# srisarya/nanopore-barcoding-ORC

Measured on AMD Instinct MI355X. Metric: Mreads/s two-round SP5×SP27 demux; % HBM roofline; 1/2/4/8 GPU, higher is better.
Workload: dtype u64

## Files before the change

nanopore-barcoding-orc_amd/csrc/dmx_kernels.hip:

```cpp
#include <algorithm>
#include <cstring>
#include <memory>
#include <type_traits>
#include <utility>
#include <vector>

#include "dmx_device.h"
#include "dmx_internal.h"

namespace dmx {

struct RoundArgs {
    Packed pk;
    const uint64_t* offs;
    const uint32_t* lens;
    const DevPanel* panel;
    const ItemView* items;
    const uint32_t* n_items_dev;
    uint32_t n_items;
    int32_t T;
    int32_t per_task_slot;
    int32_t slot_div;
    Cluster* cl;
    Outcome* outc;
    uint32_t* cl_count;
    uint32_t cl_cap;
    uint32_t* flags;
    unsigned long long* winner;
    int32_t* origin;
    int32_t* lb;
    Window* win;
    uint32_t* win_count;
    uint32_t win_cap;
    uint32_t win_scap;
    Window* win2;
    uint32_t* win2_count;
    uint32_t* diag;
    int32_t band;
    Cand* cand[2];
    uint32_t* cand_count;
    uint32_t cand_cap;
    uint32_t cand_scap;
    int32_t screen;
    Window* tasks;
    uint32_t* task_count;
    uint32_t task_cap;
    uint32_t task_scap;
    const DevPieces* pieces;
    FTask* ftask;
    uint32_t* ftask_count;
    uint32_t ftask_scap;
    uint32_t n_words;
    uint32_t nsb;
    int32_t round;
    uint32_t* cells[4];
};


struct TaskView {
    uint32_t read, n, strand, start, len;
    uint64_t off;
    int o, a;
    bool clean = false;
    uint32_t tag = 0;
    uint32_t sbl = 0;
};

template <class T>
__device__ __forceinline__ __attribute__((address_space(1))) T* sgpr_ptr(T* p) {
    const uint64_t v = reinterpret_cast<uint64_t>(p);
    const uint64_t lo = (uint32_t)__builtin_amdgcn_readfirstlane((uint32_t)v);
    const uint64_t hi = (uint32_t)__builtin_amdgcn_readfirstlane((uint32_t)(v >> 32));
    return reinterpret_cast<__attribute__((address_space(1))) T*>(lo | (hi << 32));
}

typedef unsigned int u32x4_t __attribute__((ext_vector_type(4)));
typedef unsigned int u32x2_t __attribute__((ext_vector_type(2)));
__device__ __forceinline__ void store_cand(__attribute__((address_space(1))) Cand* p, uint32_t i,
                                           const Cand& cd) {
    static_assert(sizeof(Cand) == 40, "Cand layout");
    u32x4_t a, b;
    u32x2_t c;
    __builtin_memcpy(&a, reinterpret_cast<const char*>(&cd), 16);
    __builtin_memcpy(&b, reinterpret_cast<const char*>(&cd) + 16, 16);
    __builtin_memcpy(&c, reinterpret_cast<const char*>(&cd) + 32, 8);
    auto* d = reinterpret_cast<__attribute__((address_space(1))) char*>(p + i);
    *reinterpret_cast<__attribute__((address_space(1))) u32x4_t*>(d) = a;
    *reinterpret_cast<__attribute__((address_space(1))) u32x4_t*>(d + 16) = b;
    *reinterpret_cast<__attribute__((address_space(1))) u32x2_t*>(d + 32) = c;
}

__device__ __forceinline__ void view_off(uint64_t off, TaskView& tv) {
    tv.off = off & kOffMask;
    tv.tag = 0;
    tv.sbl = 0;
}

__device__ __forceinline__ void fetch16t(const Packed& pk, const TaskView& tv, uint32_t p,
                                         uint32_t& codes, uint32_t& nbits, bool load_mask = true) {
    fetch16(pk, tv.off, tv.n, tv.strand, tv.start, p, codes, nbits, load_mask);
}

__device__ __forceinline__ bool empty_view(TaskView& tv) {
    tv.read = 0;
    tv.n = tv.start = tv.len = tv.strand = 0;
    tv.off = kMinOffset;
    tv.o = tv.a = 0;
    return false;
}

__device__ __forceinline__ bool task_view(const RoundArgs& R, uint32_t item, int sub, int A,
                                          TaskView& tv) {
    if (R.items) {
        if (!DMX_BOUND(R.pk.bd, items, item, kBufItem)) return empty_view(tv);
        const ItemView v = R.items[item];
        tv.read = v.read;
        tv.start = v.start;
        tv.len = v.len;
        tv.strand = v.strand;
        if (v.only_adapter >= 0) {
            tv.o = 0;
            tv.a = v.only_adapter;
        } else {
            tv.o = sub / A;
            tv.a = sub % A;
        }
    } else {
        tv.read = item;
        tv.start = 0;
        tv.strand = 0;
        tv.len = R.lens[item];
        tv.o = sub / A;
        tv.a = sub % A;
        if (R.per_task_slot) {
            tv.o = 0;
            tv.a = sub;
        }
    }
    if (!DMX_BOUND(R.pk.bd, reads, tv.read, kBufRead)) return empty_view(tv);
    tv.n = R.lens[tv.read];
    tv.off = R.offs[tv.read];
    if (tv.o) {
        tv.start = tv.n - tv.start - tv.len;
        tv.strand ^= 1u;
    }
    return true;
}

__device__ __forceinline__ uint32_t slot_of(const RoundArgs& R, uint32_t item, int sub) {
    if (R.per_task_slot) return item * (uint32_t)R.T + (uint32_t)sub;
    return R.slot_div ? 2u * item + (uint32_t)(sub >= R.slot_div) : item;
}

constexpr int kPeqStride = kMaxAdapters + 24;
constexpr int kIpeqStride = 9;

struct AdLite {
    int m, k, kk;
    bool front;
// ... 178 lines not shown
        __builtin_amdgcn_wave_barrier();
        if (lane == 0) *cnt = 0;
        __builtin_amdgcn_wave_barrier();
    }
};

__device__ __forceinline__ uint32_t wave_shard() {
    return (blockIdx.x * (kScanBlock / 64) + (threadIdx.x >> 6)) & (uint32_t)(kShards - 1);
}

struct ShardMap {
    uint32_t* pre;
    uint32_t scap;
    __device__ __forceinline__ void load(const uint32_t* counts, uint32_t shard_cap) {
        scap = shard_cap;
        if (threadIdx.x == 0) {
            uint32_t t = 0;
            for (int k = 0; k < kShards; ++k) {
                pre[k] = t;
                t += min(counts[k * kShardStride], shard_cap);
            }
            pre[kShards] = t;
        }
        __syncthreads();
    }
    __device__ __forceinline__ uint32_t total() const { return pre[kShards]; }
    __device__ __forceinline__ uint32_t phys(uint32_t t) const {
        uint32_t s = 0;
#pragma unroll
        for (uint32_t h = kShards / 2; h > 0; h >>= 1)
            if (t >= pre[s + h]) s += h;
        return s * scap + (t - pre[s]);
    }
};

#ifndef DMX_WAVE_CAND_CAP
#define DMX_WAVE_CAND_CAP 32
#endif
#ifndef DMX_WAVE_CAND_FLUSH
#define DMX_WAVE_CAND_FLUSH (DMX_WAVE_CAND_CAP / 2)
#endif
constexpr int kWaveCandCap = DMX_WAVE_CAND_CAP;
constexpr int kWaveWinCap = 64;

struct WaveCandSink {
    WaveStage<Cand, kWaveCandCap> st[2];
};

__device__ __forceinline__ Cand make_cand(const TaskView& tv, uint32_t item, int sub, int iend,
                                          int cost, uint32_t j) {
    Cand c;
    c.item = item;
    c.sub = (uint16_t)sub;
    c.iend = (uint8_t)iend;
    c.cost = (uint8_t)cost;
    c.j = j;
    c.n = tv.n;
    c.start = tv.start;
    c.len = tv.len;
    c.strand = (uint8_t)tv.strand;
    c.o = (uint8_t)tv.o;
    c.a = (uint8_t)tv.a;
    c.clean = tv.clean ? 1 : 0;
    c.off = tv.off | ((uint64_t)tv.tag << kOffBits);
    return c;
}

__device__ __forceinline__ bool viable_lb(int lbk, int lr, int o, int cost) {
    return beats_lb(lbk, lr - 2 * cost, o, cost);
}

template <bool MASK = true>
__device__ __forceinline__ void fetch16s(const Packed& pk, const TaskView& tv, int p,
                                         uint32_t& codes, uint32_t& nbits) {
    p = max(p, -kViewReachPre);
    if (tv.strand == 0) {
        const int64_t g = (int64_t)tv.off + (int64_t)tv.start + p;
        codes = code32(pk, g);
        nbits = (MASK && !tv.clean) ? mask32(pk, g) & 0xFFFFu : 0u;
    } else {
        const int64_t b = (int64_t)tv.off + (int64_t)tv.n - 1 - (int64_t)tv.start - p - 15;
        codes = ~rev_pairs(code32(pk, b));
        nbits = (MASK && !tv.clean) ? __brev(mask32(pk, b)) >> 16 : 0u;
    }
}

struct Chunk16 {
    uint64_t c = 0, m = 0;
};
__device__ __forceinline__ int64_t chunk16_pos(const TaskView& tv, int p) {
    p = max(p, -kViewReachPre);
    const int64_t f = (int64_t)tv.off + (int64_t)tv.start + p;
    const int64_t b = (int64_t)tv.off + (int64_t)tv.n - 1 - (int64_t)tv.start - p - 15;
    return tv.strand ? b : f;
}
__device__ __forceinline__ uint64_t load8(const uint32_t* __restrict__ w, int64_t q,
                                          const Bounds& bd, uint32_t buf) {
#ifdef DMX_DEBUG_BOUNDS
    if (!bchk(bd, q, bd.lo, bd.hi - 1, buf)) return 0ull;
#else
    (void)bd, (void)buf;
#endif
    uint64_t v;
    __builtin_memcpy(&v, w + q, 8);
    return v;
}
template <bool MASK = true>
__device__ __forceinline__ Chunk16 chunk16_load(const Packed& pk, const TaskView& tv, int p) {
    const int64_t g = chunk16_pos(tv, p);
    Chunk16 r;
    r.c = load8(pk.seq, (2 * g) >> 5, pk.bd, kBufSeq);
    if (MASK && !tv.clean) r.m = load8(pk.nmask, g >> 5, pk.bd, kBufMask);
    return r;
}
template <bool MASK = true>
__device__ __forceinline__ void chunk16_codes(const TaskView& tv, int p, const Chunk16& r,
                                              uint32_t& codes, uint32_t& nbits) {
    const int pc = max(p, -kViewReachPre);
    const uint32_t f = (uint32_t)tv.off + tv.start + (uint32_t)pc;
    const uint32_t b = (uint32_t)tv.off + tv.n - 1u - tv.start - (uint32_t)pc - 15u;
    const uint32_t g = tv.strand ? b : f;
    const uint32_t c = (uint32_t)(r.c >> ((2u * g) & 31u));
    codes = tv.strand ? ~rev_pairs(c) : c;
    if (MASK) {
        const uint32_t m = (uint32_t)(r.m >> (g & 31u));
        nbits = tv.strand ? __brev(m) >> 16 : m & 0xFFFFu;
    } else {
        nbits = 0u;
    }
}

__device__ __forceinline__ uint32_t mask32s(const Packed& pk, const TaskView& tv, int p) {
    if (tv.strand == 0) return mask32(pk, (int64_t)tv.off + (int64_t)tv.start + p);
    return __brev(mask32(pk, (int64_t)tv.off + (int64_t)tv.n - 1 - (int64_t)tv.start - p - 31));
}

template <class Sink>
__device__ __forceinline__ void flush_cands(const Sink& sink, const TaskView& tv, uint32_t item,
                                         int sub, int m, int lbk, uint32_t seg, uint64_t cm,
                                         uint64_t c0, uint64_t c1, uint64_t c2) {
    while (cm) {
        const int bit = __ffsll((unsigned long long)cm) - 1;
        cm &= cm - 1;
        const int cost = (int)((c0 >> bit) & 1ull) | ((int)((c1 >> bit) & 1ull) << 1) |
                         ((int)((c2 >> bit) & 1ull) << 2);
        const uint32_t j = seg + (uint32_t)bit;
        if (!viable_lb(lbk, min(m, (int)j + cost), tv.o, cost)) continue;
        const Cand cd = make_cand(tv, item, sub, m, cost, j);
        if (cost <= 3) sink.st[0].push(cd);
        else sink.st[1].push(cd);
    }
}

struct Bytes16 {
    uint32_t w0 = 0, w1 = 0, w2 = 0, w3 = 0;
    __device__ __forceinline__ void put(int q, uint32_t v) {
        const uint32_t sel = (0x03020100u & ~(0xFFu << (8 * (q & 3)))) | (4u << (8 * (q & 3)));
        if (q < 4) w0 = __builtin_amdgcn_perm(v, w0, sel);
        else if (q < 8) w1 = __builtin_amdgcn_perm(v, w1, sel);
        else if (q < 12) w2 = __builtin_amdgcn_perm(v, w2, sel);
        else w3 = __builtin_amdgcn_perm(v, w3, sel);
    }
    __device__ __forceinline__ int get(int q) const {
        const uint32_t x = q < 8 ? (q < 4 ? w0 : w1) : (q < 12 ? w2 : w3);
        return (int)(int8_t)(uint8_t)(x >> (8 * (q & 3)));
    }
};

struct CandOut {
    uint64_t cells = 0, c0 = 0, c1 = 0, c2 = 0;
    uint64_t rows0 = 0, rows1 = 0;
    uint64_t pv = 0, mv = 0;
    uint32_t seg = 0;
    int mlist = -1;
};

__device__ __forceinline__ uint32_t wave_sum(uint32_t v) {
#pragma unroll
    for (int d = 32; d >= 1; d >>= 1) v += __shfl_xor(v, d, 64);
    return v;
}

__device__ __forceinline__ uint32_t wave_excl_scan(uint32_t v, uint32_t& total) {
    const uint32_t lane = threadIdx.x & 63u;
    uint32_t x = v;
#pragma unroll
    for (int d = 1; d < 64; d <<= 1) {
        const uint32_t y = __shfl_up(x, d, 64);
        if (lane >= (uint32_t)d) x += y;
    }
    total = __shfl(x, 63, 64);
    return x - v;
}

__device__ __forceinline__ void emit_cands(const RoundArgs& R, const CandOut& co,
                                           const TaskView& tv, uint32_t item, int sub, int m) {
    const uint32_t n1 = (uint32_t)(__popcll(co.cells & co.c2) + __popcll(co.rows1) +
                                   (co.mlist == 1 ? 1 : 0));
    const uint32_t n0 = (uint32_t)(__popcll(co.cells & ~co.c2) + __popcll(co.rows0) +
                                   (co.mlist == 0 ? 1 : 0));
    uint32_t tot;
    const uint32_t pre = wave_excl_scan(n0 | (n1 << 16), tot);
    if (tot == 0) return;
    const uint32_t sh = wave_shard();
    uint32_t b0 = 0, b1 = 0;
    if ((threadIdx.x & 63u) == 0) {
        if (tot & 0xFFFFu) b0 = atomicAdd(R.cand_count + sh * kShardStride, tot & 0xFFFFu);
        if (tot >> 16) b1 = atomicAdd(R.cand_count + (kShards + sh) * kShardStride, tot >> 16);
    }
    b0 = __builtin_amdgcn_readfirstlane(b0) + (pre & 0xFFFFu);
    b1 = __builtin_amdgcn_readfirstlane(b1) + (pre >> 16);
    __attribute__((address_space(1))) Cand* const cl0 = sgpr_ptr(R.cand[0] + sh * R.cand_scap);
    __attribute__((address_space(1))) Cand* const cl1 = sgpr_ptr(R.cand[1] + sh * R.cand_scap);
    const auto put = [&](int l, const Cand& cd) __attribute__((always_inline)) {
        const uint32_t i = l ? b1++ : b0++;
        if (i < R.cand_scap) store_cand(l ? cl1 : cl0, i, cd);
        else atomicOr(R.flags, 8u);
    };
    uint64_t x = co.cells;
    while (x) {
        const int bit = __ffsll((unsigned long long)x) - 1;
        x &= x - 1;
        const int cost = (int)((co.c0 >> bit) & 1ull) | ((int)((co.c1 >> bit) & 1ull) << 1) |
                         ((int)((co.c2 >> bit) & 1ull) << 2);
        put(cost > 3, make_cand(tv, item, sub, m, cost, co.seg + (uint32_t)bit));
    }
    x = co.rows0 | co.rows1;
    while (x) {
        const int i = __ffsll((unsigned long long)x) - 1;
        x &= x - 1;
        const int cost = col_cost(co.pv, co.mv, i);
        put(cost > 3, make_cand(tv, item, sub, i, cost, tv.len));
    }
    if (co.mlist >= 0)
        put(co.mlist, make_cand(tv, item, sub, m, col_cost(co.pv, co.mv, m), tv.len));
}

template <int HB, class Sink>
__device__ __forceinline__ int scan_task_cand_hb(const RoundArgs& R, const Sink& sink,
                                                 const TaskView& tv, uint32_t item, int sub,
                                                 const uint64_t* peq, int A, AdLite ad,
                                                 const int8_t* acc, const int8_t* pacc,
                                                 uint32_t js, bool real, uint32_t jlo,
                                                 uint32_t jhi, bool lastcol,
                                                 CandOut* out = nullptr) {
    const int m = ad.m;
    const int kk = ad.kk;
    const bool front = ad.front;
    const uint32_t hbit = (uint32_t)(m - 1);

    uint64_t pv = (front && real) ? 0ull : ~0ull, mv = 0ull;
    int d = (front && real) ? 0 : m;
    int lbk = 0;
    bool segset = false;
    uint32_t seg = 0;
    uint64_t cm = 0, c0 = 0, c1 = 0, c2 = 0;

    auto hit = [&](uint32_t j, int dv) __attribute__((always_inline)) {
        bool ok = j >= jlo;
        int L0 = m;
        if (ok && (int)j < m + kk) {
            ok = dv <= (int)pacc[min(m, (int)j + dv)];
            L0 = min(m, (int)j - dv);
            if (ok && !(L0 >= 0 && dv <= (int)acc[L0])) L0 = -1;
        }
        if (ok) {
            if (L0 >= 0) lbk = max(lbk, lb_key(L0 - 3 * dv, tv.o, dv));
            if (!segset) {
                segset = true;
                seg = j;
            }
            const uint64_t bm = 1ull << (j - seg);
            cm |= bm;
            if (dv & 1) c0 |= bm;
            if (dv & 2) c1 |= bm;
            if (dv & 4) c2 |= bm;
        }
    };
    const int e0 = kk + 1;
    int e = d - e0;
#define DMX_CAND_REC(q)                                                                   \
    {                                                                                     \
        myers_step<HB>(eqv(q), pv, mv, e, hbit);                                          \
        hits = __builtin_amdgcn_alignbit(hits, (uint32_t)e, 31);                          \
        dq.put((q), (uint32_t)e);                                                         \
    }
#define DMX_CAND_VISIT(NQ)                                                                \
    while (hits) {                                                                        \
        const int q = (int)__clz(hits) - (32 - (NQ));                                     \
        hits &= ~(0x80000000u >> __clz(hits));                                            \
        hit(p0 + (uint32_t)q + 1u, dq.get(q) + e0);                                    \
    }
#define DMX_CAND_EQ                                                                       \
    const auto eqv = [&](int q) __attribute__((always_inline)) {                          \
        const uint32_t cq = (codes >> (2 * q)) & 3u, nq = (nb >> q) & 1u;                 \
        return peq[(cq | (nq << 2)) * kPeqStride];                                        \
    };

    uint32_t p0 = js;
    Chunk16 nx = chunk16_load(R.pk, tv, (int)p0);
    for (; p0 + 16 <= jhi; p0 += 16) {
        uint32_t codes, nb;
        chunk16_codes(tv, (int)p0, nx, codes, nb);
        if (p0 + 16 < jhi) nx = chunk16_load(R.pk, tv, (int)p0 + 16);
        if (segset && p0 + 16 >= seg + 64) {
            flush_cands(sink, tv, item, sub, m, lbk, seg, cm, c0, c1, c2);
            segset = false;
            cm = c0 = c1 = c2 = 0;
        }
        DMX_CAND_EQ
        uint32_t hits = 0;
        Bytes16 dq;
#pragma unroll
        for (int q = 0; q < 16; ++q) DMX_CAND_REC(q)
        DMX_CAND_VISIT(16)
    }
    if (p0 < jhi) {
        uint32_t codes, nb;
        chunk16_codes(tv, (int)p0, nx, codes, nb);
        if (segset && p0 + 16 >= seg + 64) {
            flush_cands(sink, tv, item, sub, m, lbk, seg, cm, c0, c1, c2);
            segset = false;
            cm = c0 = c1 = c2 = 0;
        }
        DMX_CAND_EQ
        const int cnt = (int)(jhi - p0);
        uint32_t hits = 0;
        Bytes16 dq;
#pragma unroll
        for (int q = 0; q < 16; ++q)
            if (q < cnt) DMX_CAND_REC(q)
        while (hits) {
            const int q = (int)__clz(hits) - (32 - cnt);
            hits &= ~(0x80000000u >> __clz(hits));
            hit(p0 + (uint32_t)q + 1u, dq.get(q) + e0);
        }
    }
    d = e + e0;
#undef DMX_CAND_REC
#undef DMX_CAND_VISIT
#undef DMX_CAND_EQ
    uint64_t rows = 0;
    bool mrow = false;
    const uint32_t len = tv.len;
    if (lastcol && !front) {
        int dd = 0;
        const int ilast = len == 0 ? m : m - 1;
        for (int i = 1; i <= ilast; ++i) {
            dd += (int)((pv >> (i - 1)) & 1ull) - (int)((mv >> (i - 1)) & 1ull);
            if (dd <= (int)acc[i]) {
                if (i < m) rows |= 1ull << i;
                else mrow = true;
                lbk = max(lbk, lb_key(i - 3 * dd, tv.o, dd));
            }
        }
    }
    if (out) {
        uint64_t keep = 0, x = cm;
        while (x) {
            const int bit = __ffsll((unsigned long long)x) - 1;
            x &= x - 1;
            const int cost = (int)((c0 >> bit) & 1ull) | ((int)((c1 >> bit) & 1ull) << 1) |
                             ((int)((c2 >> bit) & 1ull) << 2);
            if (viable_lb(lbk, min(m, (int)(seg + (uint32_t)bit) + cost), tv.o, cost))
                keep |= 1ull << bit;
        }
        out->cells = keep;
        out->c0 = c0;
        out->c1 = c1;
        out->c2 = c2;
        out->seg = seg;
        out->pv = pv;
        out->mv = mv;
        out->rows0 = out->rows1 = 0;
        while (rows) {
            const int i = __ffsll((unsigned long long)rows) - 1;
            rows &= rows - 1;
            const int cost = col_cost(pv, mv, i);
            if (!viable_lb(lbk, i, tv.o, cost)) continue;
            if (cost <= 3) out->rows0 |= 1ull << i;
            else out->rows1 |= 1ull << i;
        }
        out->mlist = -1;
        if (mrow) {
            const int cost = col_cost(pv, mv, m);
            if (viable_lb(lbk, m, tv.o, cost)) out->mlist = cost <= 3 ? 0 : 1;
        }
        return lbk;
    }
    if (cm) flush_cands(sink, tv, item, sub, m, lbk, seg, cm, c0, c1, c2);
    while (rows) {
        const int i = __ffsll((unsigned long long)rows) - 1;
        rows &= rows - 1;
        const int cost = col_cost(pv, mv, i);
        if (!viable_lb(lbk, i, tv.o, cost)) continue;
        const Cand cd = make_cand(tv, item, sub, i, cost, len);
        if (cost <= 3) sink.st[0].push(cd);
        else sink.st[1].push(cd);
    }
    if (mrow) {
        const int cost = col_cost(pv, mv, m);
        if (viable_lb(lbk, m, tv.o, cost)) {
            const Cand cd = make_cand(tv, item, sub, m, cost, len);
            if (cost <= 3) sink.st[0].push(cd);
            else sink.st[1].push(cd);
        }
    }
    return lbk;
}

template <class Sink>
__device__ __forceinline__ int scan_task_cand(const RoundArgs& R, const Sink& sink,
                                              const TaskView& tv, uint32_t item, int sub,
                                              const uint64_t* peq, int A, AdLite ad,
                                              const int8_t* acc, const int8_t* pacc,
                                              uint32_t js, bool real, uint32_t jlo,
                                              uint32_t jhi, bool lastcol,
                                              CandOut* out = nullptr) {
    if (ad.m > 32)
        return scan_task_cand_hb<1, Sink>(R, sink, tv, item, sub, peq, A, ad, acc, pacc, js, real,
                                          jlo, jhi, lastcol, out);
    return scan_task_cand_hb<0, Sink>(R, sink, tv, item, sub, peq, A, ad, acc, pacc, js, real, jlo,
                                      jhi, lastcol, out);
}

#define DMX_CAND_STAGE                                                                    \
    __shared__ Cand s_cand[2][kCandStageCap];                                             \
    __shared__ uint32_t s_ccnt[2], s_cbase[2];                                            \
    if (threadIdx.x < 2) s_ccnt[threadIdx.x] = 0;                                         \
    const uint32_t bsh = blockIdx.x & (uint32_t)(kShards - 1);                           \
    const CandSink sink{{Stage<Cand, kCandStageCap>{s_cand[0], &s_ccnt[0], &s_cbase[0],    \
                                                    R.cand[0] + bsh * R.cand_scap,         \
                                                    R.cand_count + bsh * kShardStride,     \
                                                    R.cand_scap,                           \
                                                    R.flags, 8u},                          \
                         Stage<Cand, kCandStageCap>{s_cand[1], &s_ccnt[1], &s_cbase[1],    \
                                                    R.cand[1] + bsh * R.cand_scap,         \
                                                    R.cand_count +                         \
                                                        (kShards + bsh) * kShardStride,    \
                                                    R.cand_scap, R.flags, 8u}}};

#define DMX_STAGES                                                                        \
    __shared__ Cluster s_cl[BAND ? 1 : kStageCap];                                        \
    __shared__ uint32_t s_clcnt, s_clbase;                                                \
    if (threadIdx.x == 0) s_clcnt = 0;                                                    \
    const Stage<Cluster> st{s_cl, &s_clcnt, &s_clbase, R.cl, R.cl_count, R.cl_cap,        \
                            R.flags, 1u};                                                 \
    __shared__ Cand s_cand[2][BAND ? kCandStageCap : 1];                                  \
    __shared__ uint32_t s_ccnt[2], s_cbase[2];                                            \
    if (threadIdx.x < 2) s_ccnt[threadIdx.x] = 0;                                         \
    const uint32_t bsh = blockIdx.x & (uint32_t)(kShards - 1);                           \
    const CandSink sink{{Stage<Cand, kCandStageCap>{s_cand[0], &s_ccnt[0], &s_cbase[0],    \
                                                    R.cand[0] + bsh * R.cand_scap,         \
                                                    R.cand_count + bsh * kShardStride,     \
                                                    R.cand_scap,                           \
                                                    R.flags, 8u},                          \
                         Stage<Cand, kCandStageCap>{s_cand[1], &s_ccnt[1], &s_cbase[1],    \
                                                    R.cand[1] + bsh * R.cand_scap,         \
                                                    R.cand_count +                         \
                                                        (kShards + bsh) * kShardStride,    \
                                                    R.cand_scap, R.flags, 8u}}};

#define DMX_CLUSTER_STAGE                                                                 \
    __shared__ Cluster s_cl[kStageCap];                                                   \
    __shared__ uint32_t s_clcnt, s_clbase;                                                \
    if (threadIdx.x == 0) s_clcnt = 0;                                                    \
    const Stage<Cluster> st{s_cl, &s_clcnt, &s_clbase, R.cl, R.cl_count, R.cl_cap,        \
                            R.flags, 1u};

template <bool BAND>
__global__ __launch_bounds__(kScanBlock) void scan_kernel(RoundArgs R) {
    __shared__ uint64_t s_peq[8 * kPeqStride];
    __shared__ int8_t s_acc[72 * kMaxAdapters];
    __shared__ int8_t s_pacc[72 * kMaxAdapters];
    __shared__ uint32_t s_amk[kMaxAdapters];
    DMX_STAGES
    load_panel_lds(R.panel, s_peq, s_acc, s_pacc, s_amk);
    __syncthreads();

    const int A = R.panel->n_adapters;
    const int T = R.T;
    const int rpb = kScanBlock / T;
    const int tid = threadIdx.x;
    const uint32_t item = blockIdx.x * (uint32_t)rpb + (uint32_t)(tid / T);
    const int sub = tid % T;
    const uint32_t n_items = R.items ? *R.n_items_dev : R.n_items;
    if (tid < rpb * T && item < n_items) {
        TaskView tv;
// ... 1897 lines not shown
                        hi |= spread_bits_nib(nb >> 8);
                    }
                    uint32_t cm0 = 0xFFFFFFFFu, cm1 = 0xFFFFFFFFu;
                    u16x2 m0 = as_pk(cm0), m1 = as_pk(cm1);
#if DMX_SCREEN_BARE
                    {
                        ScreenState ss{pv0, mv0, pv1, mv1, d0, d1, m0, m1};
                        screen_chunk<DMX_SCREEN_BARE>(qb, lo, hi, q8, qlo, ss, stale);
                        pv0 = ss.pv0, mv0 = ss.mv0, pv1 = ss.pv1, mv1 = ss.mv1;
                        d0 = ss.d0, d1 = ss.d1, m0 = ss.m0, m1 = ss.m1;
                    }
#else
                    if (__builtin_amdgcn_ballot_w64(qlo > 0) == 0) {
#pragma unroll
                        for (int c = 0; c < 16; ++c) {
                            const uint64_t e = *reinterpret_cast<const uint64_t*>(
                                qb + lds_off32(__builtin_amdgcn_ubfe(c < 8 ? lo : hi,
                                                                     4 * (c & 7), 4), q8));
                            myers_step_pk((uint32_t)e, pv0, mv0, d0);
                            myers_step_pk((uint32_t)(e >> 32), pv1, mv1, d1);
                            m0 = __builtin_elementwise_min(m0, d0);
                            m1 = __builtin_elementwise_min(m1, d1);
                        }
                    } else {
#pragma unroll
                        for (int c = 0; c < 16; ++c) {
                            const uint64_t e = *reinterpret_cast<const uint64_t*>(
                                qb + lds_off32(__builtin_amdgcn_ubfe(c < 8 ? lo : hi,
                                                                     4 * (c & 7), 4), q8));
                            myers_step_pk((uint32_t)e, pv0, mv0, d0);
                            myers_step_pk((uint32_t)(e >> 32), pv1, mv1, d1);
                            if (c >= qlo) {
                                m0 = __builtin_elementwise_min(m0, d0);
                                m1 = __builtin_elementwise_min(m1, d1);
                            }
                        }
                    }
#endif
                    cm0 = as_u32(m0);
                    cm1 = as_u32(m1);
#pragma unroll
                    for (int k = 0; k < 4; ++k) {
                        const uint32_t cmk = ((k < 2 ? cm0 : cm1) >> (16 * (k & 1))) & 0xFFFFu;
                        const int tk = max(inR ? thr[k] : -1, inE ? thre[k] : -1);
                        if (((need >> k) & 1u) && !((pass_m >> k) & 1u) && (int)cmk <= tk) {
                            pass_m |= 1u << k;
                            if (inR) end_m &= ~(1u << k);
                        }
                    }
                }
                if (lastc) {
#pragma unroll
                    for (int k = 0; k < 4; ++k) {
                        if (!((need >> k) & 1u) || ((pass_m >> k) & 1u)) continue;
                        const int a = 4 * q + k;
                        if (dPn > (int)s_pimax[a]) continue;
                        const uint32_t par = s_par[a];
                        const int l = (int)(par & 255u), lc = (int)(par >> 24);
                        const uint32_t pvh = ((k < 2 ? pv0 : pv1) >> (16 * (k & 1))) & 0xFFFFu;
                        const uint32_t mvh = ((k < 2 ? mv0 : mv1) >> (16 * (k & 1))) & 0xFFFFu;
                        bool ok = false;
                        int dd = 0;
                        for (int r = 1; r < l && !ok; ++r) {
                            if (r > l - lc) {
                                const int b = 16 - l + r - 1;
                                dd += (int)((pvh >> b) & 1u) - (int)((mvh >> b) & 1u);
                            }
                            ok = dPn + dd <= (int)s_acc[72 * a + pl + r];
                        }
                        if (ok) pass_m |= 1u << k;
                    }
                }
            }
            pass_m &= valid;
            end_m &= pass_m;
        }
        const int jr = max((int)w.j1, jsplit);
        const bool lastc = !front && w.lastcol;
#pragma unroll
        for (int k = 0; k < 4; ++k) {
            __builtin_amdgcn_wave_barrier();
            if (st.count() > kScreenCap - 64) st.flush();
            if ((near_m >> k) & 1u)
                st.push(make_task(w, 4 * q + k == 0 ? w.j1 : max(w.j1, (uint32_t)(near_sh + 1)),
                                  (uint32_t)min((int)w.j2, jsplit - 1), false, 4 * q + k));
        }
#pragma unroll
        for (int k = 0; k < 4; ++k) {
            __builtin_amdgcn_wave_barrier();
            if (st.count() > kScreenCap - 64) st.flush();
            if ((pass_m >> k) & 1u) {
                st.push(make_task(w, (uint32_t)jr, w.j2, lastc, 4 * q + k));
                if ((end_m >> k) & 1u) atomicAdd(&s_nend, 1u);
            }
        }
        __builtin_amdgcn_wave_barrier();
        if (st.count() > kScreenCap / 2) st.flush();
      }
    }
    __builtin_amdgcn_wave_barrier();
    st.flush();
    __syncthreads();
    if (threadIdx.x == 0 && s_nend) atomicAdd(&R.diag[3], s_nend);
}

template <bool BAND, class ClStage, class Sink>
__device__ __forceinline__ void wscan_task(const RoundArgs& R, const Window& w, int a, int A,
                                           const uint64_t* s_peq, const int8_t* s_acc,
                                           const int8_t* s_pacc, const uint32_t* s_amk,
                                           const ClStage& st, const Sink& sink, CandOut& co,
                                           TaskView& tv, int& sub) {
    sub = w.o * A + a;
    tv.read = 0;
    tv.n = w.n;
    tv.strand = w.strand & 1u;
    tv.clean = (w.strand & kWinClean) != 0;
    tv.start = w.start;
    tv.len = w.len;
    view_off(w.off, tv);
    tv.o = w.o;
    tv.a = a;
    const AdLite ad = ad_lite(s_amk[a]);
    int js = (int)w.j1 - ad.m - ad.k - 1;
    const bool real = js <= 0;
    if (real) js = 0;
    int lb;
    if constexpr (BAND) {
        lb = scan_task_cand(R, sink, tv, w.item, sub, s_peq + a, A, ad, s_acc + 72 * a,
                            s_pacc + 72 * a, (uint32_t)js, real, w.j1, w.j2,
                            w.lastcol != 0, &co);
    } else
        lb = scan_task(R, st, tv, w.item, sub, s_peq + a, A, ad, s_acc + 72 * a,
                       s_pacc + 72 * a, (uint32_t)js, real, w.j1, w.j2, w.lastcol != 0);
    const uint32_t slot = slot_of(R, w.item, sub);
    if (lb > 0 && DMX_BOUND(R.pk.bd, slots, slot, kBufSlot)) atomicMax(&R.lb[slot], lb);
}

#ifndef DMX_WSCAN_WAVES
#define DMX_WSCAN_WAVES 4
#endif
template <bool BAND>
__global__ __launch_bounds__(kScanBlock) __attribute__((amdgpu_waves_per_eu(DMX_WSCAN_WAVES))) void wscan_kernel(RoundArgs R) {
    __shared__ uint64_t s_peq[8 * kPeqStride];
    __shared__ int8_t s_acc[72 * kMaxAdapters];
    __shared__ int8_t s_pacc[72 * kMaxAdapters];
    __shared__ uint32_t s_amk[kMaxAdapters];
    __shared__ Cluster s_cl[BAND ? 1 : kStageCap];
    __shared__ uint32_t s_clcnt, s_clbase;
    __shared__ Cand s_wcand[BAND ? kScanBlock / 64 : 1][2][kWaveCandCap];
    __shared__ uint32_t s_wcn[kScanBlock / 64][2];
    if (threadIdx.x == 0) s_clcnt = 0;
    if (threadIdx.x < 2 * (kScanBlock / 64)) (&s_wcn[0][0])[threadIdx.x] = 0;
    const Stage<Cluster> st{s_cl, &s_clcnt, &s_clbase, R.cl, R.cl_count, R.cl_cap, R.flags, 1u};
    const uint32_t wv = BAND ? threadIdx.x >> 6 : 0u;
    const uint32_t wsh = wave_shard();
    const WaveCandSink sink{{WaveStage<Cand, kWaveCandCap>{s_wcand[wv][0], &s_wcn[wv][0],
                                                           R.cand[0] + wsh * R.cand_scap,
                                                           R.cand_count + wsh * kShardStride,
                                                           R.cand_scap,
                                                           R.flags, 8u},
                             WaveStage<Cand, kWaveCandCap>{s_wcand[wv][1], &s_wcn[wv][1],
                                                           R.cand[1] + wsh * R.cand_scap,
                                                           R.cand_count + (kShards + wsh) * kShardStride,
                                                           R.cand_scap, R.flags, 8u}}};
    load_panel_lds(R.panel, s_peq, s_acc, s_pacc, s_amk);
    __shared__ uint32_t s_spre[kShards + 1];
    ShardMap sm{s_spre, 0u};
    const Window* wl = R.panel->pre_len ? R.win2 : R.win;
    if (R.screen) sm.load(R.task_count, R.task_scap);
    else sm.load(R.panel->pre_len ? R.win2_count : R.win_count, R.win_scap);

    const int A = R.panel->n_adapters;
    if (R.screen) {
      const bool sorted = R.panel->where == kFront;
      __shared__ uint16_t s_ord[kSortGroup];
      static_assert(kSortGroup <= 65536, "sort-group indices are 16-bit");
      __shared__ uint32_t s_bin[kSortBins];
      __shared__ uint8_t s_mk[kMaxAdapters];
      for (int a = threadIdx.x; a < A; a += blockDim.x)
          s_mk[a] = (uint8_t)min(255, (int)R.panel->ad[a].m + (int)R.panel->ad[a].k + 1);
      {
        const Window* tl = R.tasks;
        const uint32_t nt = sm.total();
        for (uint32_t gb = blockIdx.x * kSortGroup; gb < nt; gb += gridDim.x * kSortGroup) {
            const uint32_t gn = min((uint32_t)kSortGroup, nt - gb);
            if (sorted) {
            if (threadIdx.x < kSortBins) s_bin[threadIdx.x] = 0;
            __syncthreads();
            constexpr int PER = kSortGroup / kScanBlock;
            uint32_t key[PER], pos[PER];
#pragma unroll
            for (int e = 0; e < PER; ++e) {
                const uint32_t li = threadIdx.x + (uint32_t)e * kScanBlock;
                const Window* w = tl + sm.phys(gb + min(li, gn - 1u));
                const int j1 = (int)w->j1, j2 = (int)w->j2, a = (int)w->info;
                const int cols = j2 - max(j1 - (int)s_mk[a], 0);
                key[e] = (uint32_t)min(max(cols, 0) >> kSortShift, kSortBins - 1);
            }
#pragma unroll
            for (int e = 0; e < PER; ++e)
                if (threadIdx.x + (uint32_t)e * kScanBlock < gn)
                    pos[e] = atomicAdd(&s_bin[key[e]], 1u);
            __syncthreads();
            if (threadIdx.x == 0) {
                uint32_t acc = 0;
                for (int b = 0; b < kSortBins; ++b) {
                    const uint32_t c = s_bin[b];
                    s_bin[b] = acc;
                    acc += c;
                }
            }
            __syncthreads();
#pragma unroll
            for (int e = 0; e < PER; ++e) {
                const uint32_t li = threadIdx.x + (uint32_t)e * kScanBlock;
                if (li < gn) s_ord[s_bin[key[e]] + pos[e]] = (uint16_t)li;
            }
            __syncthreads();
            }
            for (uint32_t sb = 0; sb < gn; sb += kScanBlock) {
                const uint32_t li = sb + threadIdx.x;
                CandOut co;
                TaskView tv{};
                int sub = 0;
                uint32_t item = 0;
                if (li < gn) {
                    const Window w = tl[sm.phys(gb + (sorted ? s_ord[li] : li))];
                    item = w.item;
                    wscan_task<BAND>(R, w, (int)w.info, A, s_peq, s_acc, s_pacc, s_amk, st, sink, co,
                                     tv, sub);
                }
                if constexpr (BAND) {
                    emit_cands(R, co, tv, item, sub, (int)(s_amk[tv.a] & 255u));
                    __builtin_amdgcn_wave_barrier();
                    if (sink.st[0].count() > DMX_WAVE_CAND_FLUSH) sink.st[0].flush();
                    if (sink.st[1].count() > DMX_WAVE_CAND_FLUSH) sink.st[1].flush();
                } else {
                    if (stage_count(&s_clcnt) > kStageCap / 2) st.flush();
                }
            }
        }
      }
        if constexpr (BAND) {
            __builtin_amdgcn_wave_barrier();
            sink.st[0].flush();
            sink.st[1].flush();
        } else {
            st.flush();
        }
        return;
    }
    const uint64_t total = (uint64_t)sm.total() * (uint64_t)A;
    for (uint64_t base = (uint64_t)blockIdx.x * blockDim.x; base < total;
         base += (uint64_t)gridDim.x * blockDim.x) {
        const uint64_t t = base + threadIdx.x;
        CandOut co;
        TaskView tv{};
        int sub = 0;
        uint32_t item = 0;
        if (t < total) {
            const Window w = wl[sm.phys((uint32_t)(t / A))];
            const int a = (int)(t % A);
            item = w.item;
            wscan_task<BAND>(R, w, a, A, s_peq, s_acc, s_pacc, s_amk, st, sink, co, tv, sub);
        }
        if constexpr (BAND) {
            emit_cands(R, co, tv, item, sub, (int)(s_amk[tv.a] & 255u));
            __builtin_amdgcn_wave_barrier();
            if (sink.st[0].count() > DMX_WAVE_CAND_FLUSH) sink.st[0].flush();
            if (sink.st[1].count() > DMX_WAVE_CAND_FLUSH) sink.st[1].flush();
        } else {
            if (stage_count(&s_clcnt) > kStageCap / 2) st.flush();
        }
    }
    if constexpr (BAND) {
        __builtin_amdgcn_wave_barrier();
        sink.st[0].flush();
        sink.st[1].flush();
    } else {
        st.flush();
    }
}

struct PeqRegs {
    uint64_t p0, p1, p2, p3;
    __device__ __forceinline__ uint64_t eq(uint32_t code) const {
        const uint64_t a = (code & 1u) ? p1 : p0;
        const uint64_t b = (code & 1u) ? p3 : p2;
        const uint64_t e = (code & 2u) ? b : a;
        return (code & 4u) ? 0ull : e;
    }
};

template <int RING>
struct Walker {
    Packed pk;
    uint32_t* flags;
    TaskView tv;
    PeqRegs peq;
    const uint64_t* rp;
    const uint64_t* rm;
    int js;
    bool real, front;

    __device__ void trace(int i, int j, int s0, int& origin, int& score) const {
        score = 0;
        int cbase = 1 << 30;
        uint32_t codes = 0, nb = 0;
        while (i > 0) {
            if (j == js) {
                if (real) {
                    if (front) {
                        origin = -i;
                    } else {
                        score -= 2 * i;
                        origin = 0;
                    }
                } else {
                    atomicOr(flags, 2u);
                    score -= 2 * i;
                    origin = js;
                }
                return;
            }
            const int p = j - 1;
            if (p < cbase) {
                cbase = max(p - 15, 0);
                fetch16t(pk, tv, (uint32_t)cbase, codes, nb);
            }
            const int sh = p - cbase;
            const uint32_t code = ((codes >> (2 * sh)) & 3u) | (((nb >> sh) & 1u) << 2);
            const int s1 = s0 == 0 ? RING - 1 : s0 - 1;
            if ((peq.eq(code) >> (i - 1)) & 1ull) {
                --i;
                --j;
                ++score;
                s0 = s1;
                continue;
            }
            const uint64_t p1 = rp[s1 * 64], m1 = rm[s1 * 64];
            const int cdel = col_cost(p1, m1, i);
            const int cd = cdel - (int)((p1 >> (i - 1)) & 1ull) + (int)((m1 >> (i - 1)) & 1ull);
            const int cins = col_cost(rp[s0 * 64], rm[s0 * 64], i - 1);
            if (cd <= cdel && cd <= cins) {
                --i;
                --j;
                score -= 1;
                s0 = s1;
            } else if (cins <= cdel) {
                --i;
                score -= 2;
            } else {
                --j;
                score -= 2;
                s0 = s1;
            }
        }
        origin = j;
    }
};

template <int RING>
__global__ __launch_bounds__(kResolveBlock) void resolve_kernel(RoundArgs R) {
    extern __shared__ __attribute__((aligned(16))) char smem[];
    uint64_t* s_rp = (uint64_t*)smem;
    uint64_t* s_rm = s_rp + RING * kResolveBlock;
    int8_t* s_acc = (int8_t*)(s_rm + RING * kResolveBlock);
    const int A = R.panel->n_adapters;
    int8_t* s_pacc = s_acc + 72 * A;
// ... 1269 lines not shown
```

Baseline: 370.5.

## Cut register pressure in scan: packed sort keys, scalarized wave ids, byte-perm getter

```diff
diff --git a/nanopore-barcoding-orc_amd/csrc/dmx_bytes16.h b/nanopore-barcoding-orc_amd/csrc/dmx_bytes16.h
--- /dev/null
+++ b/nanopore-barcoding-orc_amd/csrc/dmx_bytes16.h
@@ -0,0 +1,49 @@
+#pragma once
+#include <cstdint>
+
+#if defined(__HIPCC__)
+#define DMX_B16_FN __host__ __device__ inline __attribute__((always_inline))
+#else
+#define DMX_B16_FN inline
+#endif
+
+namespace dmx {
+
+DMX_B16_FN uint32_t byte_perm(uint32_t hi, uint32_t lo, uint32_t sel) {
+#if defined(__HIP_DEVICE_COMPILE__)
+    return __builtin_amdgcn_perm(hi, lo, sel);
+#else
+    const uint64_t src = ((uint64_t)hi << 32) | lo;
+    uint32_t r = 0;
+    for (int i = 0; i < 4; ++i) {
+        const uint32_t s = (sel >> (8 * i)) & 0xFFu;
+        uint32_t b;
+        if (s < 8) b = (uint32_t)(src >> (8 * s)) & 0xFFu;
+        else if (s < 12) b = ((src >> (16 * (s - 8) + 15)) & 1u) ? 0xFFu : 0u;
+        else b = s == 12 ? 0u : 0xFFu;
+        r |= b << (8 * i);
+    }
+    return r;
+#endif
+}
+
+#define DMX_BYTES16(name) uint32_t name##0 = 0, name##1 = 0, name##2 = 0, name##3 = 0
+#define DMX_BYTES16_ARGS(name) name##0, name##1, name##2, name##3
+
+DMX_B16_FN void bytes16_put(int q, uint32_t v, uint32_t& w0, uint32_t& w1, uint32_t& w2,
+                            uint32_t& w3) {
+    const uint32_t sel = (0x03020100u & ~(0xFFu << (8 * (q & 3)))) | (4u << (8 * (q & 3)));
+    if (q < 4) w0 = byte_perm(v, w0, sel);
+    else if (q < 8) w1 = byte_perm(v, w1, sel);
+    else if (q < 12) w2 = byte_perm(v, w2, sel);
+    else w3 = byte_perm(v, w3, sel);
+}
+
+DMX_B16_FN int bytes16_get(int q, uint32_t w0, uint32_t w1, uint32_t w2, uint32_t w3) {
+    const bool up = (q & 8) != 0;
+    const uint32_t lo = up ? w2 : w0;
+    const uint32_t hi = up ? w3 : w1;
+    return (int)(int8_t)(uint8_t)byte_perm(hi, lo, (uint32_t)q & 7u);
+}
+
+}
diff --git a/nanopore-barcoding-orc_amd/csrc/dmx_kernels.hip b/nanopore-barcoding-orc_amd/csrc/dmx_kernels.hip
--- a/nanopore-barcoding-orc_amd/csrc/dmx_kernels.hip
+++ b/nanopore-barcoding-orc_amd/csrc/dmx_kernels.hip
@@ -5,6 +5,7 @@
 #include <utility>
 #include <vector>
 
+#include "dmx_bytes16.h"
 #include "dmx_device.h"
 #include "dmx_internal.h"
 
@@ -489,20 +490,6 @@
     }
 }
 
-struct Bytes16 {
-    uint32_t w0 = 0, w1 = 0, w2 = 0, w3 = 0;
-    __device__ __forceinline__ void put(int q, uint32_t v) {
-        const uint32_t sel = (0x03020100u & ~(0xFFu << (8 * (q & 3)))) | (4u << (8 * (q & 3)));
-        if (q < 4) w0 = __builtin_amdgcn_perm(v, w0, sel);
-        else if (q < 8) w1 = __builtin_amdgcn_perm(v, w1, sel);
-        else if (q < 12) w2 = __builtin_amdgcn_perm(v, w2, sel);
-        else w3 = __builtin_amdgcn_perm(v, w3, sel);
-    }
-    __device__ __forceinline__ int get(int q) const {
-        const uint32_t x = q < 8 ? (q < 4 ? w0 : w1) : (q < 12 ? w2 : w3);
-        return (int)(int8_t)(uint8_t)(x >> (8 * (q & 3)));
-    }
-};
 
 struct CandOut {
     uint64_t cells = 0, c0 = 0, c1 = 0, c2 = 0;
@@ -620,13 +607,13 @@
     {                                                                                     \
         myers_step<HB>(eqv(q), pv, mv, e, hbit);                                          \
         hits = __builtin_amdgcn_alignbit(hits, (uint32_t)e, 31);                          \
-        dq.put((q), (uint32_t)e);                                                         \
+        bytes16_put((q), (uint32_t)e, DMX_BYTES16_ARGS(dq));                              \
     }
 #define DMX_CAND_VISIT(NQ)                                                                \
     while (hits) {                                                                        \
         const int q = (int)__clz(hits) - (32 - (NQ));                                     \
         hits &= ~(0x80000000u >> __clz(hits));                                            \
-        hit(p0 + (uint32_t)q + 1u, dq.get(q) + e0);                                    \
+        hit(p0 + (uint32_t)q + 1u, bytes16_get(q, DMX_BYTES16_ARGS(dq)) + e0);            \
     }
 #define DMX_CAND_EQ                                                                       \
     const auto eqv = [&](int q) __attribute__((always_inline)) {                          \
@@ -647,7 +634,7 @@
         }
         DMX_CAND_EQ
         uint32_t hits = 0;
-        Bytes16 dq;
+        DMX_BYTES16(dq);
 #pragma unroll
         for (int q = 0; q < 16; ++q) DMX_CAND_REC(q)
         DMX_CAND_VISIT(16)
@@ -663,14 +650,14 @@
         DMX_CAND_EQ
         const int cnt = (int)(jhi - p0);
         uint32_t hits = 0;
-        Bytes16 dq;
+        DMX_BYTES16(dq);
 #pragma unroll
         for (int q = 0; q < 16; ++q)
             if (q < cnt) DMX_CAND_REC(q)
         while (hits) {
             const int q = (int)__clz(hits) - (32 - cnt);
             hits &= ~(0x80000000u >> __clz(hits));
-            hit(p0 + (uint32_t)q + 1u, dq.get(q) + e0);
+            hit(p0 + (uint32_t)q + 1u, bytes16_get(q, DMX_BYTES16_ARGS(dq)) + e0);
         }
     }
     d = e + e0;
@@ -2874,8 +2861,8 @@
     if (threadIdx.x == 0) s_clcnt = 0;
     if (threadIdx.x < 2 * (kScanBlock / 64)) (&s_wcn[0][0])[threadIdx.x] = 0;
     const Stage<Cluster> st{s_cl, &s_clcnt, &s_clbase, R.cl, R.cl_count, R.cl_cap, R.flags, 1u};
-    const uint32_t wv = BAND ? threadIdx.x >> 6 : 0u;
-    const uint32_t wsh = wave_shard();
+    const uint32_t wv = BAND ? (uint32_t)__builtin_amdgcn_readfirstlane(threadIdx.x >> 6) : 0u;
+    const uint32_t wsh = (uint32_t)__builtin_amdgcn_readfirstlane(wave_shard());
     const WaveCandSink sink{{WaveStage<Cand, kWaveCandCap>{s_wcand[wv][0], &s_wcn[wv][0],
                                                            R.cand[0] + wsh * R.cand_scap,
                                                            R.cand_count + wsh * kShardStride,
@@ -2910,19 +2897,21 @@
             if (threadIdx.x < kSortBins) s_bin[threadIdx.x] = 0;
             __syncthreads();
             constexpr int PER = kSortGroup / kScanBlock;
-            uint32_t key[PER], pos[PER];
+            static_assert(kSortBins <= 256, "sort keys are packed as bytes");
+            uint32_t keys[(PER + 3) / 4] = {};
 #pragma unroll
             for (int e = 0; e < PER; ++e) {
                 const uint32_t li = threadIdx.x + (uint32_t)e * kScanBlock;
                 const Window* w = tl + sm.phys(gb + min(li, gn - 1u));
                 const int j1 = (int)w->j1, j2 = (int)w->j2, a = (int)w->info;
                 const int cols = j2 - max(j1 - (int)s_mk[a], 0);
-                key[e] = (uint32_t)min(max(cols, 0) >> kSortShift, kSortBins - 1);
+                const uint32_t key = (uint32_t)min(max(cols, 0) >> kSortShift, kSortBins - 1);
+                keys[e >> 2] |= key << (8 * (e & 3));
             }
 #pragma unroll
             for (int e = 0; e < PER; ++e)
                 if (threadIdx.x + (uint32_t)e * kScanBlock < gn)
-                    pos[e] = atomicAdd(&s_bin[key[e]], 1u);
+                    atomicAdd(&s_bin[(keys[e >> 2] >> (8 * (e & 3))) & 255u], 1u);
             __syncthreads();
             if (threadIdx.x == 0) {
                 uint32_t acc = 0;
@@ -2936,7 +2925,9 @@
 #pragma unroll
             for (int e = 0; e < PER; ++e) {
                 const uint32_t li = threadIdx.x + (uint32_t)e * kScanBlock;
-                if (li < gn) s_ord[s_bin[key[e]] + pos[e]] = (uint16_t)li;
+                if (li < gn)
+                    s_ord[atomicAdd(&s_bin[(keys[e >> 2] >> (8 * (e & 3))) & 255u], 1u)] =
+                        (uint16_t)li;
             }
             __syncthreads();
             }
```

Result: no change. 374.2 (median of 6 runs) (+1.0%).
